# Snowdar/asv-subtools

Hardware: NVIDIA H100
Metric: frames/sec x-vector extraction (80-d fbank) (higher is better)
Workload: dtype f32 (bf16x3 split operands on wgmma, fp32 accumulate in registers)

## Files before the change

### asv_subtools_b200/csrc/ptx.cuh

```cuda
#pragma once
#include <cuda_runtime.h>
#include <cuda.h>
#include <stdint.h>

namespace xvb {

#ifndef XVB_WATCHDOG
#define XVB_WATCHDOG 1
#endif

__device__ __forceinline__ uint32_t smem_u32(const void* p) {
  return static_cast<uint32_t>(__cvta_generic_to_shared(p));
}

__device__ __forceinline__ uint32_t lane_id() {
  uint32_t l;
  asm volatile("mov.u32 %0, %%laneid;" : "=r"(l));
  return l;
}

__device__ __forceinline__ bool elect_one() {
  uint32_t pred = 0;
  asm volatile(
      "{\n\t"
// ... 48 lines not shown
      : "=r"(ok)
      : "r"(smem_u32(bar)), "r"(parity), "r"(1000000u)
      : "memory");
  return ok != 0;
}
__device__ __forceinline__ void mbar_wait(uint64_t* bar, uint32_t parity) {
#if XVB_WATCHDOG
  uint32_t spins = 0;
  while (!mbar_try_wait(bar, parity)) {
    if (++spins > 4000u) {
#if XVB_WATCHDOG >= 2
      printf("xvb: mbarrier watchdog: block %d thread %d bar@%u parity %u\n", (int)blockIdx.x, (int)threadIdx.x,
             smem_u32(bar), parity);
#endif
      __trap();
    }
  }
#else
  while (!mbar_try_wait(bar, parity)) {
  }
#endif
}

__device__ __forceinline__ void tma_prefetch_desc(const CUtensorMap* m) {
  asm volatile("prefetch.tensormap [%0];" ::"l"(reinterpret_cast<uint64_t>(m)) : "memory");
}
__device__ __forceinline__ void tma_load_2d(void* smem, const CUtensorMap* m, uint64_t* bar, int c0, int c1) {
  asm volatile(
      "cp.async.bulk.tensor.2d.shared::cluster.global.mbarrier::complete_tx::bytes [%0], [%1, {%3, %4}], [%2];" ::"r"(
          smem_u32(smem)),
      "l"(reinterpret_cast<uint64_t>(m)), "r"(smem_u32(bar)), "r"(c0), "r"(c1)
      : "memory");
}
__device__ __forceinline__ void tma_load_3d(void* smem, const CUtensorMap* m, uint64_t* bar, int c0, int c1, int c2) {
  asm volatile(
      "cp.async.bulk.tensor.3d.shared::cluster.global.mbarrier::complete_tx::bytes [%0], [%1, {%3, %4, %5}], [%2];" ::
          "r"(smem_u32(smem)),
      "l"(reinterpret_cast<uint64_t>(m)), "r"(smem_u32(bar)), "r"(c0), "r"(c1), "r"(c2)
      : "memory");
}
__device__ __forceinline__ void tma_load_4d(void* smem, const CUtensorMap* m, uint64_t* bar, int c0, int c1, int c2, int c3) {
  asm volatile(
      "cp.async.bulk.tensor.4d.shared::cluster.global.mbarrier::complete_tx::bytes [%0], [%1, {%3, %4, %5, %6}], [%2];" ::
          "r"(smem_u32(smem)),
      "l"(reinterpret_cast<uint64_t>(m)), "r"(smem_u32(bar)), "r"(c0), "r"(c1), "r"(c2), "r"(c3)
      : "memory");
}
__device__ __forceinline__ void tma_store_3d(const CUtensorMap* m, uint32_t smem_addr, int c0, int c1, int c2) {
  asm volatile("cp.async.bulk.tensor.3d.global.shared::cta.bulk_group [%0, {%2, %3, %4}], [%1];" ::"l"(
                   reinterpret_cast<uint64_t>(m)),
               "r"(smem_addr), "r"(c0), "r"(c1), "r"(c2)
               : "memory");
}
__device__ __forceinline__ void tma_store_commit() { asm volatile("cp.async.bulk.commit_group;" ::: "memory"); }
template <int kPending>
__device__ __forceinline__ void tma_store_wait_read() {
  asm volatile("cp.async.bulk.wait_group.read %0;" ::"n"(kPending) : "memory");
}
template <int kPending>
__device__ __forceinline__ void tma_store_wait_done() {
  asm volatile("cp.async.bulk.wait_group %0;" ::"n"(kPending) : "memory");
}
__device__ __forceinline__ void st_shared_u32(uint32_t addr, uint32_t v) {
  asm volatile("st.shared.b32 [%0], %1;" ::"r"(addr), "r"(v) : "memory");
}
__device__ __forceinline__ float2 ld_shared_f2(uint32_t addr) {
  float2 v;
  asm volatile("ld.shared.v2.f32 {%0, %1}, [%2];" : "=f"(v.x), "=f"(v.y) : "r"(addr));
  return v;
}
__device__ __forceinline__ void wgmma_fence() { asm volatile("wgmma.fence.sync.aligned;" ::: "memory"); }
__device__ __forceinline__ void wgmma_commit() { asm volatile("wgmma.commit_group.sync.aligned;" ::: "memory"); }
template <int kPending>
__device__ __forceinline__ void wgmma_wait() {
  asm volatile("wgmma.wait_group.sync.aligned %0;" ::"n"(kPending) : "memory");
}
template <uint32_t kRegs>
__device__ __forceinline__ void setmaxnreg_dec() { asm volatile("setmaxnreg.dec.sync.aligned.u32 %0;" ::"n"(kRegs)); }
template <uint32_t kRegs>
__device__ __forceinline__ void setmaxnreg_inc() { asm volatile("setmaxnreg.inc.sync.aligned.u32 %0;" ::"n"(kRegs)); }
template <int R>
__device__ __forceinline__ void wgmma_fence_operands(float (&d)[R]) {
#pragma unroll
  for (int i = 0; i < R; ++i) asm volatile("" : "+f"(d[i])::"memory");
}

template <int N>
__device__ __forceinline__ void wgmma_bf16(float (&d)[N / 2], uint64_t desc_a, uint64_t desc_b, uint32_t scale_d);
template <>
__device__ __forceinline__ void wgmma_bf16<32>(float (&d)[16], uint64_t desc_a, uint64_t desc_b, uint32_t scale_d) {
  asm volatile(
      "{\n\t.reg .pred p;\n\tsetp.ne.b32 p, %18, 0;\n\t"
      "wgmma.mma_async.sync.aligned.m64n32k16.f32.bf16.bf16 {%0, %1, %2, %3, %4, %5, %6, %7, %8, %9, %10, %11, %12, %13, %14, %15}, %16, %17, p, 1, 1, 0, 0;\n\t}\n"
      : "+f"(d[0]), "+f"(d[1]), "+f"(d[2]), "+f"(d[3]), "+f"(d[4]), "+f"(d[5]), "+f"(d[6]), "+f"(d[7]), "+f"(d[8]), "+f"(d[9]), "+f"(d[10]), "+f"(d[11]), "+f"(d[12]), "+f"(d[13]), "+f"(d[14]), "+f"(d[15])
      : "l"(desc_a), "l"(desc_b), "r"(scale_d));
}
template <>
__device__ __forceinline__ void wgmma_bf16<64>(float (&d)[32], uint64_t desc_a, uint64_t desc_b, uint32_t scale_d) {
  asm volatile(
      "{\n\t.reg .pred p;\n\tsetp.ne.b32 p, %34, 0;\n\t"
      "wgmma.mma_async.sync.aligned.m64n64k16.f32.bf16.bf16 {%0, %1, %2, %3, %4, %5, %6, %7, %8, %9, %10, %11, %12, %13, %14, %15, %16, %17, %18, %19, %20, %21, %22, %23, %24, %25, %26, %27, %28, %29, %30, %31}, %32, %33, p, 1, 1, 0, 0;\n\t}\n"
      : "+f"(d[0]), "+f"(d[1]), "+f"(d[2]), "+f"(d[3]), "+f"(d[4]), "+f"(d[5]), "+f"(d[6]), "+f"(d[7]), "+f"(d[8]), "+f"(d[9]), "+f"(d[10]), "+f"(d[11]), "+f"(d[12]), "+f"(d[13]), "+f"(d[14]), "+f"(d[15]), "+f"(d[16]), "+f"(d[17]), "+f"(d[18]), "+f"(d[19]), "+f"(d[20]), "+f"(d[21]), "+f"(d[22]), "+f"(d[23]), "+f"(d[24]), "+f"(d[25]), "+f"(d[26]), "+f"(d[27]), "+f"(d[28]), "+f"(d[29]), "+f"(d[30]), "+f"(d[31])
      : "l"(desc_a), "l"(desc_b), "r"(scale_d));
}
template <>
__device__ __forceinline__ void wgmma_bf16<128>(float (&d)[64], uint64_t desc_a, uint64_t desc_b, uint32_t scale_d) {
// ... 18 lines not shown
```

### asv_subtools_b200/csrc/tdnn_gemm.cu

```cuda
#include <cuda.h>
#include <cuda_bf16.h>
#include <cuda_runtime.h>

#include <stdlib.h>

#include <mutex>

#include "common.cuh"
#include "ptx.cuh"

namespace xvb {

constexpr int kBlockM = 128;
constexpr int kBlockK = 64;
constexpr int kABytes = kBlockM * kBlockK * 2;
constexpr int kNumConsumers = 256;
constexpr int kProducerWarp = kNumConsumers / 32;
constexpr int kSlabBytes = 16384;
constexpr int kStagePlaneBytes = 64 * kBlockK * 2;
constexpr int kStageOutBytes = 2 * kStagePlaneBytes;
constexpr int kCoefBytes = 3 * kBlockK * 4;
constexpr int kEpiBytes = 2 * (kStageOutBytes + kCoefBytes);
static_assert(kEpiBytes >= kSlabBytes, "the histogram slab lives in the epilogue region");

template <int BLOCK_N, bool kHist, bool kSwish>
__host__ __device__ constexpr bool ping_pong() { return BLOCK_N == 128 && !kHist && !kSwish; }
template <int BLOCK_N, bool kHist, bool kSwish>
__host__ __device__ constexpr int gemm_threads() { return kNumConsumers + (ping_pong<BLOCK_N, kHist, kSwish>() ? 128 : 32); }
constexpr uint32_t kProducerRegs = 40, kConsumerRegs = 232;

struct TdnnGemmParams {
  int B, T, Cin, Cout;
  int Tb, Bb, num_t_blk, num_b_blk, num_n_blk, num_tiles;
  int ntaps, cin_p16, num_cblk;
  int ctx[XVB_MAX_TAPS];
  int flags;
  const float* bias;
  const float* scale;
  const float* shift;
  const float* row_bias;
  const float* utt_bias;
  long long ld_utt;
  int log2_tb;
  float* pool_partial;
  int num_src;
  int unit_first, unit_stride;
  unsigned long long* hist;
  const int* row_label;
  const int* col_label;
  float hist_lo, hist_inv_w;
  int hist_bins;
  int hist_sym;
  int hist_group, num_units;
  int k_slices, kb_per_slice;
  int group_ng, group_kg;
  int out_T;
  const int* lengths;
  int tma_store;
#ifdef XVB_TILE_TIMELINE
  unsigned long long* timeline;
  int timeline_tiles;
  int timeline_general;
#endif
  __nv_bfloat16* y_hi;
  __nv_bfloat16* y_lo;
  long long ldy;
  float* y_f32;
  long long ldyf;
};

template <int BLOCK_N, bool kPool, bool kHist>
__host__ __device__ constexpr bool staged_epilogue() { return !kPool && !kHist && BLOCK_N % kBlockK == 0; }

template <int BLOCK_N, bool kStagedEpi>
struct GemmCfg {
  static constexpr int kTailBytes = kStagedEpi ? kEpiBytes : kSlabBytes;
  static constexpr int kBBytes = BLOCK_N * kBlockK * 2;
  static constexpr int kStageBytes = 2 * kABytes + 2 * kBBytes;
  static constexpr int kStages = (192 * 1024) / kStageBytes > 6 ? 6 : (192 * 1024) / kStageBytes;
  static constexpr int kAccRegs = BLOCK_N / 2;
  static constexpr int kSmemBytes = kStages * kStageBytes + kTailBytes + 1024  + 256 ;
  static_assert(kSmemBytes <= 232448, "exceeds the 227 KB shared memory of an sm_90 CTA");
  static_assert(kStages >= 2, "need at least a double-buffered operand pipeline");
};

template <bool kHist>
__device__ __forceinline__ bool decode_tile(const TdnnGemmParams& p, int tile, int& m_unit, int& n_blk, int& slice) {
  slice = 0;
  if constexpr (!kHist) {
    if (p.k_slices > 1) { slice = tile % p.k_slices; tile /= p.k_slices; }
    m_unit = p.unit_first + (tile / p.num_n_blk) * p.unit_stride;
    n_blk = tile % p.num_n_blk;
    return true;
  } else {
    const int per_band = p.num_n_blk * p.hist_group;
    const int band = tile / per_band, r = tile - band * per_band;
    n_blk = r / p.hist_group;
    const int mi = band * p.hist_group + (r - n_blk * p.hist_group);
    m_unit = 2 * (p.unit_first + (mi >> 1) * p.unit_stride) + (mi & 1);
    return mi < 2 * p.num_units && !(p.hist_sym && n_blk < m_unit);
  }
}

__device__ __forceinline__ void chan_merge(float& n, float& mean, float& m2, float nb, float meanb, float m2b) {
  const float tot = n + nb;
  if (tot > 0.f) {
    const float d = meanb - mean, wb = nb / tot;
    mean = fmaf(d, wb, mean);
    m2 += m2b + d * d * n * wb;
  }
  n = tot;
}

__device__ __noinline__ float epi_tanh(float v) { return tanhf(v); }
__device__ __noinline__ float epi_sigmoid(float v) { return 1.f / (1.f + expf(-v)); }

__device__ __noinline__ void epi_zero_row(const TdnnGemmParams& p, long long grow, long long frow, int c_begin, int c_end) {
  for (int c = c_begin; c < c_end; c += 8) {
    const bool has1 = c + 1 < p.Cout;
    if (p.y_hi) {
      if (has1) {
        *reinterpret_cast<uint32_t*>(p.y_hi + grow * p.ldy + c) = 0u;
        *reinterpret_cast<uint32_t*>(p.y_lo + grow * p.ldy + c) = 0u;
      } else {
        p.y_hi[grow * p.ldy + c] = __float2bfloat16(0.f);
        p.y_lo[grow * p.ldy + c] = __float2bfloat16(0.f);
      }
    }
    if (p.y_f32) {
      float* df = p.y_f32 + frow * p.ldyf + c;
      if (has1) *reinterpret_cast<float2*>(df) = make_float2(0.f, 0.f);
      else *df = 0.f;
    }
  }
}

#ifdef XVB_TILE_TIMELINE
#define XVB_TL(...) __VA_ARGS__
constexpr int kTimelineHead = 8, kTimelineRec = 8;
static unsigned long long* g_timeline = nullptr;
static int g_timeline_tiles = 0;
static bool g_timeline_direct = false;
__device__ __forceinline__ unsigned long long global_timer() {
  unsigned long long t;
  asm volatile("mov.u64 %0, %%globaltimer;" : "=l"(t));
  return t;
}
#else
#define XVB_TL(...)
#endif

template <int BLOCK_N, bool kPool, bool kHist, bool kSwish = false>
__global__ void __launch_bounds__(gemm_threads<BLOCK_N, kHist, kSwish>(), 1)
tdnn_gemm_bf16x3_kernel(const __grid_constant__ CUtensorMap map_a_hi, const __grid_constant__ CUtensorMap map_a_lo,
                        const __grid_constant__ CUtensorMap map_a2_hi, const __grid_constant__ CUtensorMap map_a2_lo,
                        const __grid_constant__ CUtensorMap map_w_hi, const __grid_constant__ CUtensorMap map_w_lo,
                        const __grid_constant__ CUtensorMap map_y_hi, const __grid_constant__ CUtensorMap map_y_lo,
                        const __grid_constant__ TdnnGemmParams p) {
  constexpr bool kStaged = staged_epilogue<BLOCK_N, kPool, kHist>();
  using Cfg = GemmCfg<BLOCK_N, kStaged>;
  constexpr int kStages = Cfg::kStages;
  constexpr int kBBytes = Cfg::kBBytes;
  constexpr int kStageBytes = Cfg::kStageBytes;
  static_assert(!kPool || BLOCK_N == kBlockM, "fused pooling: 128 channels x 128 frames per tile");
  constexpr bool kPingPong = ping_pong<BLOCK_N, kHist, kSwish>();
  constexpr int kHalves = kPingPong ? 2 : 1;
  constexpr int kReleaseWarps = kPingPong ? 4 : kNumConsumers / 32;

  extern __shared__ uint8_t smem_raw[];
  uint8_t* smem = reinterpret_cast<uint8_t*>((reinterpret_cast<uintptr_t>(smem_raw) + 1023) & ~uintptr_t(1023));
  uint8_t* slab_base = smem + kStages * kStageBytes;
  uint64_t* full_bar = reinterpret_cast<uint64_t*>(slab_base + Cfg::kTailBytes);
  uint64_t* empty_bar = full_bar + kStages;

  const int warp = threadIdx.x >> 5;
  const int lane = threadIdx.x & 31;

  if (warp == kProducerWarp && lane == 0) {
    tma_prefetch_desc(&map_a_hi);
    tma_prefetch_desc(&map_a_lo);
    tma_prefetch_desc(&map_w_hi);
    tma_prefetch_desc(&map_w_lo);
    if (kStaged && p.tma_store) {
      tma_prefetch_desc(&map_y_hi);
      tma_prefetch_desc(&map_y_lo);
    }
    for (int i = 0; i < kStages; ++i) {
      mbar_init(&full_bar[i], 1);
      mbar_init(&empty_bar[i], kReleaseWarps);
    }
    fence_barrier_init();
  }
  __syncthreads();
  asm volatile("griddepcontrol.wait;" ::: "memory");
  asm volatile("fence.proxy.async;" ::: "memory");

  const int num_kblk = p.num_src * p.ntaps * p.num_cblk;

  if (warp >= kProducerWarp) {
    if constexpr (kPingPong) setmaxnreg_dec<kProducerRegs>();
    if (warp == kProducerWarp && lane == 0) {
      int stage = 0;
      uint32_t phase = 0;
      for (int tile = blockIdx.x; tile < p.num_tiles; tile += gridDim.x) {
        int m_unit, n_blk, slice;
        if (!decode_tile<kHist>(p, tile, m_unit, n_blk, slice)) continue;
        const int cb_begin = slice * p.kb_per_slice;
        const int cb_end = p.k_slices > 1 ? min(p.num_cblk, cb_begin + p.kb_per_slice) : p.num_cblk;
        const int b0 = (m_unit / p.num_t_blk) * p.Bb, t0 = (m_unit % p.num_t_blk) * p.Tb;
        const int n0 = n_blk * BLOCK_N;
        const int a_c0 = p.group_ng ? (n0 / p.group_ng) * p.group_kg : 0;
        for (int src = 0; src < p.num_src; ++src) {
          const CUtensorMap* ma_hi = src == 0 ? &map_a_hi : &map_a2_hi;
          const CUtensorMap* ma_lo = src == 0 ? &map_a_lo : &map_a2_lo;
          for (int tap = 0; tap < p.ntaps; ++tap) {
            const int tt = t0 + p.ctx[tap];
            for (int cb = cb_begin; cb < cb_end; ++cb) {
              mbar_wait(&empty_bar[stage], phase ^ 1);
              uint8_t* s = smem + stage * kStageBytes;
              const int kw = tap * p.cin_p16 + cb * kBlockK;
              mbar_expect_tx(&full_bar[stage], kStageBytes);
              tma_load_3d(s, ma_hi, &full_bar[stage], a_c0 + cb * kBlockK, tt, b0);
              tma_load_3d(s + kABytes, ma_lo, &full_bar[stage], a_c0 + cb * kBlockK, tt, b0);
              tma_load_2d(s + 2 * kABytes, &map_w_hi, &full_bar[stage], kw, n0);
              tma_load_2d(s + 2 * kABytes + kBBytes, &map_w_lo, &full_bar[stage], kw, n0);
              if (++stage == kStages) { stage = 0; phase ^= 1; }
            }
          }
        }
      }
    }
    return;
  }

  if constexpr (kPingPong) setmaxnreg_inc<kConsumerRegs>();
  const int wg = warp >> 2;
  const int q4 = lane & 3;
  const int row_base = kPingPong ? 0 : 64 * wg;
  const int row0 = row_base + 16 * (warp & 3) + (lane >> 2);
  const int etid = threadIdx.x;
  const bool relu = (p.flags & XVB_RELU) != 0;
  const bool bn = (p.flags & XVB_BN) != 0;
  const bool act_sigmoid = (p.flags & XVB_SIGMOID) != 0;
  const bool act_tanh = (p.flags & XVB_TANH) != 0;
  const float relu_floor = relu ? 0.f : -INFINITY;
  float acc[kHalves][Cfg::kAccRegs];
#pragma unroll
  for (int hh = 0; hh < kHalves; ++hh)
#pragma unroll
    for (int i = 0; i < Cfg::kAccRegs; ++i) acc[hh][i] = 0.f;
  auto half_down = [&]() {
#pragma unroll
    for (int i = 0; i < Cfg::kAccRegs; ++i) acc[0][i] = acc[kHalves - 1][i];
  };
  int stage = 0;
  uint32_t phase = 0;
  uint32_t it = 0;

  uint32_t h_below[2] = {0u, 0u}, h_above[2] = {0u, 0u};
  const uint32_t hslab = smem_u32(slab_base);
  auto hist_flush = [&]() {
    asm volatile("bar.sync 1, 256;" ::: "memory");
#pragma unroll
    for (int c = 0; c < 2; ++c) {
      if (h_below[c]) asm volatile("red.shared.add.u32 [%0], %1;" ::"r"(hslab + (c * p.hist_bins) * 4), "r"(h_below[c]) : "memory");
      if (h_above[c]) asm volatile("red.shared.add.u32 [%0], %1;" ::"r"(hslab + (c * p.hist_bins + p.hist_bins - 1) * 4), "r"(h_above[c]) : "memory");
      h_below[c] = 0u; h_above[c] = 0u;
    }
    asm volatile("bar.sync 1, 256;" ::: "memory");
    for (int e = etid; e < 2 * p.hist_bins; e += kNumConsumers) {
      uint32_t c;
      asm volatile("ld.shared.u32 %0, [%1];" : "=r"(c) : "r"(hslab + e * 4) : "memory");
      if (c) {
        atomicAdd(p.hist + e, (unsigned long long)c);
        asm volatile("st.shared.u32 [%0], %1;" ::"r"(hslab + e * 4), "r"(0u) : "memory");
      }
    }
    asm volatile("bar.sync 1, 256;" ::: "memory");
  };
  if constexpr (kHist) {
    for (int e = etid; e < 2 * p.hist_bins; e += kNumConsumers)
      asm volatile("st.shared.u32 [%0], %1;" ::"r"(hslab + e * 4), "r"(0u) : "memory");
    asm volatile("bar.sync 1, 256;" ::: "memory");
  }

  XVB_TL(
    long long tl_start = 0, tl_first = 0, tl_issued = 0, tl_retired = 0, tl_wait = 0;
    unsigned long long* tl_cta = p.timeline ? p.timeline + (size_t)blockIdx.x * (kTimelineHead + (size_t)kTimelineRec * p.timeline_tiles) : nullptr;
    if (tl_cta && threadIdx.x == 0) { tl_cta[0] = global_timer(); tl_cta[1] = (unsigned long long)clock64(); }
  )
  int tj = 0;
  XVB_TL(auto tl_flush = [&]() {
    if (tl_cta && (threadIdx.x & 127) == 0 && tj < p.timeline_tiles) {
      unsigned long long* r = tl_cta + kTimelineHead + (size_t)kTimelineRec * tj;
      r[0] = (unsigned long long)tl_start; r[1] = (unsigned long long)tl_first; r[2] = (unsigned long long)tl_issued;
      r[3] = (unsigned long long)tl_retired; r[4] = (unsigned long long)clock64(); r[5] = (unsigned long long)tl_wait;
      r[6] = (unsigned long long)wg; r[7] = 1ull;
    }
  };)
  for (int tile = blockIdx.x; tile < p.num_tiles; tile += gridDim.x, ++tj) {
    int m_unit, n_blk, slice;
    if (!decode_tile<kHist>(p, tile, m_unit, n_blk, slice)) continue;
    int kb_begin = 0, kb_end = num_kblk;
    if (p.k_slices > 1) {
      kb_begin = slice * p.kb_per_slice;
      kb_end = min(num_kblk, kb_begin + p.kb_per_slice);
    }
    if constexpr (kPingPong) {
      if ((tj & 1) != wg) {
        stage += kb_end - kb_begin;
        phase ^= (uint32_t)(stage / kStages) & 1u;
        stage %= kStages;
        continue;
      }
      if (tj > 0) asm volatile("bar.sync %0, 256;" ::"r"(2 + wg) : "memory");
    }
    ++it;
    XVB_TL(tl_start = clock64(); tl_wait = 0;)
    auto stage_before = [&]() { return stage == 0 ? kStages - 1 : stage - 1; };
    for (int kb = kb_begin; kb < kb_end; ++kb) {
      XVB_TL(const long long tl_w0 = clock64();)
      mbar_wait(&full_bar[stage], phase);
      XVB_TL(const long long tl_w1 = clock64(); tl_wait += tl_w1 - tl_w0; tl_first = kb == kb_begin ? tl_w1 : tl_first;)
      const uint32_t sa = smem_u32(smem + stage * kStageBytes);
      const uint64_t dx_hi = make_sw128_desc(sa), dx_lo = make_sw128_desc(sa + kABytes);
      const uint64_t dw_hi = make_sw128_desc(sa + 2 * kABytes), dw_lo = make_sw128_desc(sa + 2 * kABytes + kBBytes);
      const uint64_t da_hi = kPool ? dw_hi : dx_hi, da_lo = kPool ? dw_lo : dx_lo;
      const uint64_t db_hi = kPool ? dx_hi : dw_hi, db_lo = kPool ? dx_lo : dw_lo;
      wgmma_fence();
#pragma unroll
      for (int s = 0; s < kBlockK / 16; ++s) {
        const uint64_t koff = (uint64_t)(s * 32 >> 4);
#pragma unroll
        for (int hh = 0; hh < kHalves; ++hh) {
          const uint64_t m_off = (uint64_t)((row_base + 64 * hh) * 128 >> 4);
          wgmma_bf16<BLOCK_N>(acc[hh], da_lo + m_off + koff, db_hi + koff, s == 0 ? (uint32_t)(kb != kb_begin) : 1u);
          wgmma_bf16<BLOCK_N>(acc[hh], da_hi + m_off + koff, db_lo + koff, 1);
          wgmma_bf16<BLOCK_N>(acc[hh], da_hi + m_off + koff, db_hi + koff, 1);
        }
      }
      wgmma_commit();
      wgmma_wait<1>();
      if (kb != kb_begin && lane == 0) mbar_arrive(&empty_bar[stage_before()]);
      if (++stage == kStages) { stage = 0; phase ^= 1; }
    }
    if (kPingPong && tile + gridDim.x < p.num_tiles) asm volatile("bar.arrive %0, 256;" ::"r"(3 - wg) : "memory");
    XVB_TL(tl_issued = clock64();)
    wgmma_wait<0>();
    XVB_TL(tl_retired = clock64();)
#pragma unroll
    for (int hh = 0; hh < kHalves; ++hh) wgmma_fence_operands(acc[hh]);
    if (kb_end > kb_begin && lane == 0) mbar_arrive(&empty_bar[stage_before()]);

    const int b0 = (m_unit / p.num_t_blk) * p.Bb, t0 = (m_unit % p.num_t_blk) * p.Tb;
    const int n0 = n_blk * BLOCK_N;

    if constexpr (kPool) {
      int nv = p.T - t0;
      nv = nv < 0 ? 0 : (nv > p.Tb ? p.Tb : nv);
      const int tblk = m_unit % p.num_t_blk;
      const int gl = p.Tb < 8 ? p.Tb : 8;
#pragma unroll 1
      for (int hh = 0; hh < kHalves; ++hh) {
      if (hh > 0) half_down();
      int b0h = b0, nvh = nv;
      asm volatile("" : "+r"(b0h), "+r"(nvh));
      if (p.Tb == 8 && nvh == 8 XVB_TL(&& !p.timeline_general)) {
#pragma unroll
        for (int h = 0; h < 2; ++h) {
          const int cch = n0 + row0 + 64 * hh + 8 * h;
          const bool cvalid = cch < p.Cout;
          const float bias_c = (cvalid && p.bias) ? __ldg(p.bias + cch) : 0.f;
          const float scale_c = (cvalid && bn) ? __ldg(p.scale + cch) : 1.f;
          const float shift_c = (cvalid && bn) ? __ldg(p.shift + cch) : 0.f;
          float* dst0 = p.pool_partial + ((long long)tblk * p.B + b0h) * (2LL * p.Cout) + cch;
          const bool writer = cvalid && q4 == 0;
#pragma unroll
          for (int i = 0; i < BLOCK_N / 8; ++i) {
            const float x0 = fmaf(fmaxf(acc[0][4 * i + 2 * h] + bias_c, relu_floor), scale_c, shift_c);
            const float x1 = fmaf(fmaxf(acc[0][4 * i + 2 * h + 1] + bias_c, relu_floor), scale_c, shift_c);
            float mean = 0.5f * (x0 + x1) + 0.f;
            float m2 = 0.5f * (x0 - x1) * (x0 - x1);
            float d = __shfl_xor_sync(0xffffffffu, mean, 1) - mean;
            float m2b = __shfl_xor_sync(0xffffffffu, m2, 1);
            mean = fmaf(d, 0.5f, mean);
            m2 += m2b + d * d * 2.f * 0.5f;
            d = __shfl_xor_sync(0xffffffffu, mean, 2) - mean;
            m2b = __shfl_xor_sync(0xffffffffu, m2, 2);
            mean = fmaf(d, 0.5f, mean);
            m2 += m2b + d * d * 4.f * 0.5f;
            if (writer && b0h + i < p.B) {
              float* dst = dst0 + (long long)i * (2LL * p.Cout);
              dst[0] = mean;
              dst[p.Cout] = m2;
            }
          }
        }
        continue;
      }
#pragma unroll
      for (int h = 0; h < 2; ++h) {
        const int cch = n0 + row0 + 64 * hh + 8 * h;
        const bool cvalid = cch < p.Cout;
        const float bias_c = (cvalid && p.bias) ? __ldg(p.bias + cch) : 0.f;
        const float scale_c = (cvalid && bn) ? __ldg(p.scale + cch) : 1.f;
        const float shift_c = (cvalid && bn) ? __ldg(p.shift + cch) : 0.f;
        auto emit = [&](int col, float mean, float m2) {
          const int bb = b0h + (col >> p.log2_tb);
          if (cvalid && bb < p.B) {
            float* dst = p.pool_partial + ((long long)tblk * p.B + bb) * (2LL * p.Cout) + cch;
            dst[0] = mean;
            dst[p.Cout] = m2;
          }
        };
        float rn = 0.f, rmean = 0.f, rm2 = 0.f;
#pragma unroll
        for (int i = 0; i < BLOCK_N / 8; ++i) {
          const int col = 8 * i + 2 * q4;
          const float x0 = fmaf(fmaxf(acc[0][4 * i + 2 * h] + bias_c, relu_floor), scale_c, shift_c);
          const float x1 = fmaf(fmaxf(acc[0][4 * i + 2 * h + 1] + bias_c, relu_floor), scale_c, shift_c);
          if (p.Tb == 1) {
            if (nvh > 0) { emit(col, x0, 0.f); emit(col + 1, x1, 0.f); }
            continue;
          }
          const int j = col & (p.Tb - 1);
          const bool v0 = j < nvh, v1 = j + 1 < nvh;
          const float pn = (float)v0 + (float)v1;
          const float pm = v1 ? 0.5f * (x0 + x1) : (v0 ? x0 : 0.f);
          const float pm2 = v1 ? 0.5f * (x0 - x1) * (x0 - x1) : 0.f;
          chan_merge(rn, rmean, rm2, pn, pm, pm2);
          if (((col - 2 * q4 + 8) & (p.Tb - 1)) == 0) {
            if (gl >= 4) chan_merge(rn, rmean, rm2, __shfl_xor_sync(0xffffffffu, rn, 1),
                                    __shfl_xor_sync(0xffffffffu, rmean, 1), __shfl_xor_sync(0xffffffffu, rm2, 1));
            if (gl >= 8) chan_merge(rn, rmean, rm2, __shfl_xor_sync(0xffffffffu, rn, 2),
                                    __shfl_xor_sync(0xffffffffu, rmean, 2), __shfl_xor_sync(0xffffffffu, rm2, 2));
            if (((2 * q4) & (gl - 1)) == 0 && rn > 0.f) emit(col & ~(p.Tb - 1), rmean, rm2);
            rn = 0.f; rmean = 0.f; rm2 = 0.f;
          }
        }
      }
      }
      XVB_TL(tl_flush();)
      continue;
    }

    if constexpr (kHist) {
      const float top = (float)(p.hist_bins - 2);
#pragma unroll
      for (int h = 0; h < 2; ++h) {
        const int row = row0 + 8 * h;
        const int b = b0 + (row >> p.log2_tb), t = t0 + (row & (p.Tb - 1));
        const bool valid = (b < p.B) && (t < p.T);
        const float rbias = (p.row_bias && valid) ? __ldg(p.row_bias + (long long)b * p.T + t) : 0.f;
        const int lab_r = valid ? __ldg(p.row_label + b) : -1;
#pragma unroll
        for (int i = 0; i < BLOCK_N / 8; ++i) {
#pragma unroll
          for (int e = 0; e < 2; ++e) {
            const int c = n0 + 8 * i + 2 * q4 + e;
            const bool in = c < p.Cout;
            const uint32_t ok = (valid && in && (!p.hist_sym || c > b)) ? 1u : 0u;
            const float sc = acc[0][4 * i + 2 * h + e] + ((in && p.bias) ? __ldg(p.bias + c) : 0.f) + rbias;
            const float x = (sc - p.hist_lo) * p.hist_inv_w;
            const uint32_t cls = (in && __ldg(p.col_label + c) == lab_r) ? 1u : 0u;
            const uint32_t bl = x < 0.f ? ok : 0u;
            const uint32_t ab = !(x < top) ? ok : 0u;
            h_below[0] += bl & (cls ^ 1u); h_below[1] += bl & cls;
            h_above[0] += ab & (cls ^ 1u); h_above[1] += ab & cls;
            if (ok & ~(bl | ab))
              asm volatile("red.shared.add.u32 [%0], %1;" ::"r"(hslab + ((int)cls * p.hist_bins + 1 + (int)x) * 4), "r"(1u) : "memory");
          }
        }
      }
      if ((it & 0x3fffu) == 0) hist_flush();
      continue;
    }

    if constexpr (kStaged) {
      if (p.tma_store) {
        int tid = threadIdx.x;
        asm volatile("" : "+r"(tid));
        const int wgo = tid >> 7, wtid = tid & 127, q4o = tid & 3;
        const int prow = 16 * ((tid >> 5) & 3) + ((tid & 31) >> 2);
        const uint32_t stg = smem_u32(slab_base) + wgo * kStageOutBytes;
        const uint32_t coefs = smem_u32(slab_base) + 2 * kStageOutBytes + wgo * kCoefBytes;
        const int ebar = 4 + wgo;
        const uint32_t coef = coefs + 8 * q4o;
        const uint32_t my = stg + (uint32_t)prow * 128u + ((uint32_t)(prow & 7) << 4) + 4u * q4o;
#pragma unroll 1
        for (int hh = 0; hh < kHalves; ++hh) {
          if (hh > 0) half_down();
          const int hrow = (kPingPong ? 0 : 64 * wgo) + 64 * hh;
          uint32_t keep[2];
#pragma unroll
          for (int r = 0; r < 2; ++r) {
            const int row = hrow + prow + 8 * r;
            const int b = b0 + (row >> p.log2_tb), t = t0 + (row & (p.Tb - 1));
            keep[r] = (p.lengths && b < p.B && t >= __ldg(p.lengths + b)) ? 0u : 0xffffffffu;
          }
#pragma unroll
          for (int cr = 0; cr < BLOCK_N / kBlockK; ++cr) {
            const int c0 = n0 + kBlockK * cr;
            if (c0 >= p.Cout) break;
            if (wtid == 0) tma_store_wait_read<0>();
            if (wtid < kBlockK) {
              const int c = c0 + wtid;
              const bool in = c < p.Cout;
              st_shared_f32(coefs + 4 * wtid, (in && p.bias) ? __ldg(p.bias + c) : 0.f);
              st_shared_f32(coefs + 4 * (kBlockK + wtid), (in && bn) ? __ldg(p.scale + c) : 1.f);
              st_shared_f32(coefs + 4 * (2 * kBlockK + wtid), (in && bn) ? __ldg(p.shift + c) : 0.f);
            }
            asm volatile("bar.sync %0, 128;" ::"r"(ebar) : "memory");
#pragma unroll
            for (int i = 0; i < kBlockK / 8; ++i) {
              const float2 bias_c = ld_shared_f2(coef + 32 * i), scale_c = ld_shared_f2(coef + 32 * i + 4 * kBlockK),
                           shift_c = ld_shared_f2(coef + 32 * i + 8 * kBlockK);
              const float bias_e[2] = {bias_c.x, bias_c.y}, scale_e[2] = {scale_c.x, scale_c.y},
                          shift_e[2] = {shift_c.x, shift_c.y};
#pragma unroll
              for (int r = 0; r < 2; ++r) {
                float x[2] = {acc[0][4 * (8 * cr + i) + 2 * r], acc[0][4 * (8 * cr + i) + 2 * r + 1]};
#pragma unroll
                for (int e = 0; e < 2; ++e) {
                  float v = x[e] + bias_e[e] + 0.f;
                  v = fmaxf(v, relu_floor);
                  if constexpr (kSwish) v = v / (1.f + expf(-v));
                  if (bn) v = fmaf(v, scale_e[e], shift_e[e]);
                  if (act_tanh) v = epi_tanh(v);
                  if (act_sigmoid) v = epi_sigmoid(v);
                  x[e] = v;
                }
                __nv_bfloat16 h0, l0, h1, l1;
                split_bf16(x[0], h0, l0);
                split_bf16(x[1], h1, l1);
                const uint32_t at = (my ^ ((uint32_t)i << 4)) + 1024u * r;
                st_shared_u32(at, pack_bf16x2(h0, h1) & keep[r]);
                st_shared_u32(at + kStagePlaneBytes, pack_bf16x2(l0, l1) & keep[r]);
              }
            }
            fence_proxy_async();
            asm volatile("bar.sync %0, 128;" ::"r"(ebar) : "memory");
            if (wtid == 0) {
              const int hb = b0 + (hrow >> p.log2_tb), ht = t0 + (hrow & (p.Tb - 1));
              tma_store_3d(&map_y_hi, stg, c0, ht, hb);
              tma_store_3d(&map_y_lo, stg + kStagePlaneBytes, c0, ht, hb);
              tma_store_commit();
            }
          }
        }
        XVB_TL(tl_flush();)
        continue;
      }
    }
    if constexpr (!kPool && !kHist) {
#pragma unroll 1
      for (int hh = 0; hh < kHalves; ++hh) {
      if (hh > 0) half_down();
      constexpr int kRows = 2;
      bool live[kRows];
      float rbias[kRows];
      const float* ub[kRows];
      long long grow[kRows], frow[kRows];
#pragma unroll
      for (int r = 0; r < kRows; ++r) {
        const int row = row0 + 64 * hh + 8 * r;
        const int b = b0 + (row >> p.log2_tb), t = t0 + (row & (p.Tb - 1));
        live[r] = b < p.B && t < p.T;
        grow[r] = (long long)b * p.T + t;
        frow[r] = (long long)b * p.out_T + t + slice;
        if (live[r] && p.lengths && t >= __ldg(p.lengths + b)) {
          epi_zero_row(p, grow[r], frow[r], n0 + 2 * q4, min(n0 + BLOCK_N, p.Cout));
          live[r] = false;
        }
        rbias[r] = (live[r] && p.row_bias) ? __ldg(p.row_bias + grow[r]) : 0.f;
        ub[r] = (live[r] && p.utt_bias) ? p.utt_bias + (long long)b * p.ld_utt : nullptr;
      }
#pragma unroll
      for (int i = 0; i < BLOCK_N / 8; ++i) {
        const int c = n0 + 8 * i + 2 * q4;
        if (c >= p.Cout) break;
        const bool has1 = c + 1 < p.Cout;
        float bias_c[2], scale_c[2], shift_c[2];
#pragma unroll
        for (int e = 0; e < 2; ++e) {
          const bool in = e == 0 || has1;
          bias_c[e] = (in && p.bias) ? __ldg(p.bias + c + e) : 0.f;
          scale_c[e] = (in && bn) ? __ldg(p.scale + c + e) : 1.f;
          shift_c[e] = (in && bn) ? __ldg(p.shift + c + e) : 0.f;
        }
#pragma unroll
        for (int r = 0; r < kRows; ++r) {
          if (!live[r]) continue;
          float x[2] = {acc[0][4 * i + 2 * r], acc[0][4 * i + 2 * r + 1]};
#pragma unroll
          for (int e = 0; e < 2; ++e) {
            if (e == 1 && !has1) break;
            float v = x[e] + bias_c[e] + rbias[r];
            if (ub[r]) v += __ldg(ub[r] + c + e);
            v = fmaxf(v, relu_floor);
            if constexpr (kSwish) v = v / (1.f + expf(-v));
            if (bn) v = fmaf(v, scale_c[e], shift_c[e]);
            if (act_tanh) v = epi_tanh(v);
            if (act_sigmoid) v = epi_sigmoid(v);
            x[e] = v;
          }
          if (p.y_hi) {
            __nv_bfloat16 h0, l0, h1, l1;
            split_bf16(x[0], h0, l0);
            split_bf16(x[1], h1, l1);
            __nv_bfloat16* dh = p.y_hi + grow[r] * p.ldy + c;
            __nv_bfloat16* dl = p.y_lo + grow[r] * p.ldy + c;
            if (has1) {
              *reinterpret_cast<uint32_t*>(dh) = pack_bf16x2(h0, h1);
              *reinterpret_cast<uint32_t*>(dl) = pack_bf16x2(l0, l1);
            } else {
              *dh = h0;
              *dl = l0;
            }
          }
          if (p.y_f32) {
            float* df = p.y_f32 + frow[r] * p.ldyf + c;
            if (has1) *reinterpret_cast<float2*>(df) = make_float2(x[0], x[1]);
            else *df = x[0];
          }
        }
      }
      }
      XVB_TL(tl_flush();)
    }
  }
  if constexpr (kHist) hist_flush();
  if constexpr (kStaged) {
    if (p.tma_store && (threadIdx.x & 127) == 0) tma_store_wait_done<0>();
  }
  XVB_TL(if (tl_cta && (threadIdx.x & 127) == 0) { tl_cta[2 + 2 * wg] = global_timer(); tl_cta[3 + 2 * wg] = (unsigned long long)clock64(); })
}

__global__ void segment_reduce_kernel(const float* __restrict__ part, int S, int B, int Cout, const float* __restrict__ bias,
                                      const float* __restrict__ scale, const float* __restrict__ shift, int flags,
                                      float* __restrict__ y_f32, long long ldyf, __nv_bfloat16* __restrict__ y_hi,
                                      __nv_bfloat16* __restrict__ y_lo, long long ldy) {
  asm volatile("griddepcontrol.wait;" ::: "memory");
  const long long idx = blockIdx.x * (long long)blockDim.x + threadIdx.x;
  if (idx >= (long long)B * Cout) return;
  const int b = (int)(idx / Cout), c = (int)(idx - (long long)b * Cout);
  const float* src = part + (long long)b * S * Cout + c;
  float x = src[0];
  for (int s = 1; s < S; ++s) x += src[(long long)s * Cout];
  x += bias ? bias[c] : 0.f;
  if (flags & XVB_RELU) x = fmaxf(x, 0.f);
  if (flags & XVB_BN) x = fmaf(x, scale[c], shift[c]);
  if (flags & XVB_TANH) x = tanhf(x);
  if (flags & XVB_SIGMOID) x = 1.f / (1.f + expf(-x));
  if (y_f32) y_f32[(long long)b * ldyf + c] = x;
  if (y_hi) {
    __nv_bfloat16 h, l;
    split_bf16(x, h, l);
    y_hi[(long long)b * ldy + c] = h;
    y_lo[(long long)b * ldy + c] = l;
  }
}

typedef CUresult (*PFN_encodeTiled)(CUtensorMap*, CUtensorMapDataType, cuuint32_t, void*, const cuuint64_t*,
                                    const cuuint64_t*, const cuuint32_t*, const cuuint32_t*, CUtensorMapInterleave,
                                    CUtensorMapSwizzle, CUtensorMapL2promotion, CUtensorMapFloatOOBfill);

static PFN_encodeTiled get_encode() {
  static PFN_encodeTiled fn = nullptr;
  static std::once_flag once;
  std::call_once(once, [] {
    void* p = nullptr;
    cudaDriverEntryPointQueryResult q;
    if (cudaGetDriverEntryPoint("cuTensorMapEncodeTiled", &p, cudaEnableDefault, &q) == cudaSuccess &&
        q == cudaDriverEntryPointSuccess)
      fn = reinterpret_cast<PFN_encodeTiled>(p);
  });
  return fn;
}

int make_tensor_map(CUtensorMap* m, const void* base, int esize, int rank, const unsigned long long* dims,
                    const unsigned long long* strides_bytes, const unsigned* box, int swizzle_bytes) {
  PFN_encodeTiled enc = get_encode();
  if (!enc) { set_error("cuTensorMapEncodeTiled entry point not available"); return XVB_ECUDA; }
  cuuint64_t d[5], st[4];
  cuuint32_t bx[5], es[5];
  for (int i = 0; i < rank; ++i) { d[i] = dims[i]; bx[i] = box[i]; es[i] = 1; }
  for (int i = 0; i + 1 < rank; ++i) st[i] = strides_bytes[i];
  const CUtensorMapSwizzle sw = swizzle_bytes == 128 ? CU_TENSOR_MAP_SWIZZLE_128B
                               : swizzle_bytes == 64 ? CU_TENSOR_MAP_SWIZZLE_64B : CU_TENSOR_MAP_SWIZZLE_NONE;
  CUresult r = enc(m, esize == 2 ? CU_TENSOR_MAP_DATA_TYPE_BFLOAT16 : CU_TENSOR_MAP_DATA_TYPE_FLOAT32, rank,
                   const_cast<void*>(base), d, st, bx, es, CU_TENSOR_MAP_INTERLEAVE_NONE, sw,
                   CU_TENSOR_MAP_L2_PROMOTION_L2_256B, CU_TENSOR_MAP_FLOAT_OOB_FILL_NONE);
  if (r != CUDA_SUCCESS) { set_error("cuTensorMapEncodeTiled(rank %d) failed: %d", rank, (int)r); return XVB_ECUDA; }
  return XVB_OK;
}

static int make_frame_map(CUtensorMap* m, const void* base, int C, int T, int B, long long ld, int Tb, int Bb,
                          long long batch_stride = 0) {
  PFN_encodeTiled enc = get_encode();
  if (!enc) { set_error("cuTensorMapEncodeTiled entry point not available"); return XVB_ECUDA; }
  cuuint64_t dims[3] = {(cuuint64_t)C, (cuuint64_t)T, (cuuint64_t)B};
  cuuint64_t strides[2] = {(cuuint64_t)ld * 2, batch_stride ? (cuuint64_t)batch_stride * 2 : (cuuint64_t)ld * 2 * (cuuint64_t)T};
  cuuint32_t box[3] = {(cuuint32_t)kBlockK, (cuuint32_t)Tb, (cuuint32_t)Bb};
  cuuint32_t estr[3] = {1, 1, 1};
  CUresult r = enc(m, CU_TENSOR_MAP_DATA_TYPE_BFLOAT16, 3, const_cast<void*>(base), dims, strides, box, estr,
                   CU_TENSOR_MAP_INTERLEAVE_NONE, CU_TENSOR_MAP_SWIZZLE_128B, CU_TENSOR_MAP_L2_PROMOTION_L2_256B,
                   CU_TENSOR_MAP_FLOAT_OOB_FILL_NONE);
  if (r != CUDA_SUCCESS) { set_error("cuTensorMapEncodeTiled(frame map C=%d T=%d B=%d ld=%lld) failed: %d", C, T, B, ld, (int)r); return XVB_ECUDA; }
  return XVB_OK;
}

static int make_store_map(CUtensorMap* m, const void* base, int Cout, int T, int B, long long ld, int Tb) {
  const int box_t = Tb < 64 ? Tb : 64;
  const unsigned long long dims[3] = {(unsigned long long)Cout, (unsigned long long)T, (unsigned long long)B};
  const unsigned long long strides[2] = {(unsigned long long)ld * 2, (unsigned long long)ld * 2 * (unsigned long long)T};
  const unsigned box[3] = {(unsigned)kBlockK, (unsigned)box_t, (unsigned)(64 / box_t)};
  return make_tensor_map(m, base, 2, 3, dims, strides, box, 128);
}

static int make_weight_map(CUtensorMap* m, const void* base, long long K, int Cout, int block_n) {
  PFN_encodeTiled enc = get_encode();
  if (!enc) { set_error("cuTensorMapEncodeTiled entry point not available"); return XVB_ECUDA; }
  cuuint64_t dims[2] = {(cuuint64_t)K, (cuuint64_t)Cout};
  cuuint64_t strides[1] = {(cuuint64_t)K * 2};
  cuuint32_t box[2] = {(cuuint32_t)kBlockK, (cuuint32_t)block_n};
  cuuint32_t estr[2] = {1, 1};
  CUresult r = enc(m, CU_TENSOR_MAP_DATA_TYPE_BFLOAT16, 2, const_cast<void*>(base), dims, strides, box, estr,
                   CU_TENSOR_MAP_INTERLEAVE_NONE, CU_TENSOR_MAP_SWIZZLE_128B, CU_TENSOR_MAP_L2_PROMOTION_L2_256B,
                   CU_TENSOR_MAP_FLOAT_OOB_FILL_NONE);
  if (r != CUDA_SUCCESS) { set_error("cuTensorMapEncodeTiled(weight map K=%lld Cout=%d) failed: %d", K, Cout, (int)r); return XVB_ECUDA; }
  return XVB_OK;
}

static void choose_m_tile(int B, int T, int* Tb_out, int* Bb_out, int max_tb = 128) {
  if (T == 1) {
    *Tb_out = 1;
    *Bb_out = 128;
    return;
  }
  long long best = -1;
  int bt = max_tb;
  for (int Tb = max_tb; Tb >= 1; Tb >>= 1) {
    const int Bb = 128 / Tb;
    const long long rows = (long long)((T + Tb - 1) / Tb) * Tb * ((B + Bb - 1) / Bb) * Bb;
    if (best < 0 || rows < best) { best = rows; bt = Tb; }
  }
  *Tb_out = bt;
  *Bb_out = 128 / bt;
}

struct GemmPlan {
  CUtensorMap ma_hi, ma_lo, ma2_hi, ma2_lo, mw_hi, mw_lo, my_hi, my_lo;
  TdnnGemmParams p;
  int (*launch)(const GemmPlan&, const TdnnGemmParams&, cudaStream_t) = nullptr;
  int grid = 0;
  int pdl = 1;
  bool reduce = false;
  const float* r_bias = nullptr; const float* r_scale = nullptr; const float* r_shift = nullptr;
  int r_flags = 0;
  float* r_y_f32 = nullptr; long long r_ldyf = 0;
  __nv_bfloat16* r_y_hi = nullptr; __nv_bfloat16* r_y_lo = nullptr; long long r_ldy = 0;
};

template <int BLOCK_N, bool kPool, bool kHist, bool kSwish>
static int launch_inst(const GemmPlan& pl, const TdnnGemmParams& p, cudaStream_t stream) {
  using Cfg = GemmCfg<BLOCK_N, staged_epilogue<BLOCK_N, kPool, kHist>()>;
  XVB_ENSURE_DYN_SMEM((tdnn_gemm_bf16x3_kernel<BLOCK_N, kPool, kHist, kSwish>), Cfg::kSmemBytes);
  cudaLaunchConfig_t cfg{};
  cfg.gridDim = dim3(pl.grid);
  cfg.blockDim = dim3(gemm_threads<BLOCK_N, kHist, kSwish>());
  cfg.dynamicSmemBytes = Cfg::kSmemBytes;
  cfg.stream = stream;
  cudaLaunchAttribute attr[1];
  attr[0].id = cudaLaunchAttributeProgrammaticStreamSerialization;
  attr[0].val.programmaticStreamSerializationAllowed = 1;
  cfg.attrs = attr;
  cfg.numAttrs = pl.pdl ? 1 : 0;
  XVB_CUDA(cudaLaunchKernelEx(&cfg, tdnn_gemm_bf16x3_kernel<BLOCK_N, kPool, kHist, kSwish>, pl.ma_hi, pl.ma_lo, pl.ma2_hi,
                              pl.ma2_lo, pl.mw_hi, pl.mw_lo, pl.my_hi, pl.my_lo, p));
  XVB_LAUNCH_CHECK();
  return XVB_OK;
}

template <int BLOCK_N, bool kPool = false, bool kHist = false, bool kSwish = false>
static int prepare_gemm(GemmPlan& pl, const void* w_hi, const void* w_lo) {
  TdnnGemmParams& p = pl.p;
  const long long K = (long long)p.ntaps * p.cin_p16;
  int rc = make_weight_map(&pl.mw_hi, w_hi, K, p.Cout, BLOCK_N);
  if (rc) return rc;
  rc = make_weight_map(&pl.mw_lo, w_lo, K, p.Cout, BLOCK_N);
  if (rc) return rc;
  p.num_n_blk = (p.Cout + BLOCK_N - 1) / BLOCK_N;
  p.tma_store = staged_epilogue<BLOCK_N, kPool, kHist>() && p.y_hi && !p.y_f32 && p.k_slices == 1 && !p.row_bias && !p.utt_bias &&
                p.Cout % 8 == 0;
  XVB_TL(if (g_timeline_direct) p.tma_store = 0;)
  if (p.tma_store) {
    if ((rc = make_store_map(&pl.my_hi, p.y_hi, p.Cout, p.T, p.B, p.ldy, p.Tb))) return rc;
    if ((rc = make_store_map(&pl.my_lo, p.y_lo, p.Cout, p.T, p.B, p.ldy, p.Tb))) return rc;
  } else {
    pl.my_hi = pl.mw_hi; pl.my_lo = pl.mw_lo;
  }
  const int all_m_units = kHist ? (p.num_t_blk * p.num_b_blk + 1) / 2 : p.num_t_blk * p.num_b_blk;
  if (p.unit_first >= all_m_units) { pl.launch = nullptr; return XVB_OK; }
  const int num_m_units = (all_m_units - p.unit_first + p.unit_stride - 1) / p.unit_stride;
  p.num_units = num_m_units;
  p.hist_group = 8;
  const long long tiles = kHist ? (long long)((2 * num_m_units + p.hist_group - 1) / p.hist_group) * p.hist_group * p.num_n_blk
                                : (long long)num_m_units * p.num_n_blk * (p.k_slices > 1 ? p.k_slices : 1);
  XVB_CHECK_ARG(tiles < (1ll << 31), "xvb_tdnn_affine: %d x %d tiles exceed one launch", num_m_units, p.num_n_blk);
  p.num_tiles = (int)tiles;
  p.out_T = p.k_slices > 1 ? p.k_slices : p.T;
  const int sms = sm_count();
  pl.grid = p.num_tiles < sms ? p.num_tiles : sms;
  static const int pdl = getenv("XVB_PDL") ? atoi(getenv("XVB_PDL")) : 1;
  pl.pdl = pdl;
  pl.launch = &launch_inst<BLOCK_N, kPool, kHist, kSwish>;
  return XVB_OK;
}

static int splitk_slices(const xvb_tdnn_args_t& a, bool has_hist, int* kb_per_slice) {
  const int num_cblk = (a.Cin + kBlockK - 1) / kBlockK;
  *kb_per_slice = num_cblk;
  const int splitk = getenv("XVB_SPLITK") ? atoi(getenv("XVB_SPLITK")) : 1;
  if (!(splitk && a.T == 1 && a.ntaps == 1 && !a.x2_hi && !a.pool_partial && !has_hist && !a.row_bias && !a.utt_bias &&
        !(a.flags & XVB_SWISH) && a.groups <= 1 &&
        a.B <= 1024 && num_cblk >= 24 && a.Cout % 4 == 0))
    return 1;
  int S = num_cblk / 6;
  S = S > 8 ? 8 : S;
  *kb_per_slice = (num_cblk + S - 1) / S;
  return (num_cblk + *kb_per_slice - 1) / *kb_per_slice;
}

}

using namespace xvb;

size_t xvb::gemm_plan_scratch_bytes(const xvb_tdnn_args_t& a, const TrialHist* th) {
  int kb;
  const int S = splitk_slices(a, th != nullptr, &kb);
  return S > 1 ? (size_t)a.B * S * a.Cout * sizeof(float) : 0;
}

int xvb::gemm_plan_build(GemmPlan** out, const xvb_tdnn_args_t& a, const TrialHist* th, void* scratch) {
  int rc = require_sm90();
  if (rc) return rc;
  *out = nullptr;
  const int B = a.B, T = a.T, Cin = a.Cin, Cout = a.Cout, ntaps = a.ntaps;
  XVB_CHECK_ARG(a.x_hi && a.x_lo && a.w_hi && a.w_lo, "xvb_tdnn_affine: null operand pointer");
// ... 204 lines not shown
```

Baseline: 34.48 million.

## Stage pooling partial statistics in shared memory and write them with TMA stores

The pooling epilogue (Tb==8) now writes per-tile mean/M2 partials into the shared-memory epilogue slab instead of scattering them to global memory from individual threads. One thread per warpgroup then issues a 4D bulk tensor store through a new tensor map over the pool_partial buffer. This replaces many strided scalar global stores with one async bulk copy per tile, at the cost of extra shared memory for the pooling variant and extra barrier and store-wait synchronisation. Timeline instrumentation records epilogue phase times when the timeline build flag is on.

```diff
diff --git a/asv_subtools_b200/csrc/ptx.cuh b/asv_subtools_b200/csrc/ptx.cuh
--- a/asv_subtools_b200/csrc/ptx.cuh
+++ b/asv_subtools_b200/csrc/ptx.cuh
@@ -124,6 +124,12 @@
                "r"(smem_addr), "r"(c0), "r"(c1), "r"(c2)
                : "memory");
 }
+__device__ __forceinline__ void tma_store_4d(const CUtensorMap* m, uint32_t smem_addr, int c0, int c1, int c2, int c3) {
+  asm volatile("cp.async.bulk.tensor.4d.global.shared::cta.bulk_group [%0, {%2, %3, %4, %5}], [%1];" ::"l"(
+                   reinterpret_cast<uint64_t>(m)),
+               "r"(smem_addr), "r"(c0), "r"(c1), "r"(c2), "r"(c3)
+               : "memory");
+}
 __device__ __forceinline__ void tma_store_commit() { asm volatile("cp.async.bulk.commit_group;" ::: "memory"); }
 template <int kPending>
 __device__ __forceinline__ void tma_store_wait_read() {
diff --git a/asv_subtools_b200/csrc/tdnn_gemm.cu b/asv_subtools_b200/csrc/tdnn_gemm.cu
--- a/asv_subtools_b200/csrc/tdnn_gemm.cu
+++ b/asv_subtools_b200/csrc/tdnn_gemm.cu
@@ -72,9 +72,9 @@
 template <int BLOCK_N, bool kPool, bool kHist>
 __host__ __device__ constexpr bool staged_epilogue() { return !kPool && !kHist && BLOCK_N % kBlockK == 0; }
 
-template <int BLOCK_N, bool kStagedEpi>
+template <int BLOCK_N, bool kPool, bool kHist>
 struct GemmCfg {
-  static constexpr int kTailBytes = kStagedEpi ? kEpiBytes : kSlabBytes;
+  static constexpr int kTailBytes = (staged_epilogue<BLOCK_N, kPool, kHist>() || kPool) ? kEpiBytes : kSlabBytes;
   static constexpr int kBBytes = BLOCK_N * kBlockK * 2;
   static constexpr int kStageBytes = 2 * kABytes + 2 * kBBytes;
   static constexpr int kStages = (192 * 1024) / kStageBytes > 6 ? 6 : (192 * 1024) / kStageBytes;
@@ -137,7 +137,7 @@
 
 #ifdef XVB_TILE_TIMELINE
 #define XVB_TL(...) __VA_ARGS__
-constexpr int kTimelineHead = 8, kTimelineRec = 8;
+constexpr int kTimelineHead = 8, kTimelineRec = 12;
 static unsigned long long* g_timeline = nullptr;
 static int g_timeline_tiles = 0;
 static bool g_timeline_direct = false;
@@ -158,7 +158,7 @@
                         const __grid_constant__ CUtensorMap map_y_hi, const __grid_constant__ CUtensorMap map_y_lo,
                         const __grid_constant__ TdnnGemmParams p) {
   constexpr bool kStaged = staged_epilogue<BLOCK_N, kPool, kHist>();
-  using Cfg = GemmCfg<BLOCK_N, kStaged>;
+  using Cfg = GemmCfg<BLOCK_N, kPool, kHist>;
   constexpr int kStages = Cfg::kStages;
   constexpr int kBBytes = Cfg::kBBytes;
   constexpr int kStageBytes = Cfg::kStageBytes;
@@ -181,7 +181,7 @@
     tma_prefetch_desc(&map_a_lo);
     tma_prefetch_desc(&map_w_hi);
     tma_prefetch_desc(&map_w_lo);
-    if (kStaged && p.tma_store) {
+    if ((kStaged || kPool) && p.tma_store) {
       tma_prefetch_desc(&map_y_hi);
       tma_prefetch_desc(&map_y_lo);
     }
@@ -286,6 +286,9 @@
 
   XVB_TL(
     long long tl_start = 0, tl_first = 0, tl_issued = 0, tl_retired = 0, tl_wait = 0;
+    long long tl_ep[4] = {0, 0, 0, 0};
+    long long tl_t = 0;
+    auto tl_mark = [&](int ph) { const long long t = clock64(); tl_ep[ph] += t - tl_t; tl_t = t; };
     unsigned long long* tl_cta = p.timeline ? p.timeline + (size_t)blockIdx.x * (kTimelineHead + (size_t)kTimelineRec * p.timeline_tiles) : nullptr;
     if (tl_cta && threadIdx.x == 0) { tl_cta[0] = global_timer(); tl_cta[1] = (unsigned long long)clock64(); }
   )
@@ -296,6 +299,7 @@
       r[0] = (unsigned long long)tl_start; r[1] = (unsigned long long)tl_first; r[2] = (unsigned long long)tl_issued;
       r[3] = (unsigned long long)tl_retired; r[4] = (unsigned long long)clock64(); r[5] = (unsigned long long)tl_wait;
       r[6] = (unsigned long long)wg; r[7] = 1ull;
+      for (int ph = 0; ph < 4; ++ph) r[8 + ph] = (unsigned long long)tl_ep[ph];
     }
   };)
   for (int tile = blockIdx.x; tile < p.num_tiles; tile += gridDim.x, ++tj) {
@@ -313,10 +317,13 @@
         stage %= kStages;
         continue;
       }
-      if (tj > 0) asm volatile("bar.sync %0, 256;" ::"r"(2 + wg) : "memory");
+      if (tj > 0) {
+        if (kPool && (threadIdx.x & 127) == 0) tma_store_wait_read<0>();
+        asm volatile("bar.sync %0, 256;" ::"r"(2 + wg) : "memory");
+      }
     }
     ++it;
-    XVB_TL(tl_start = clock64(); tl_wait = 0;)
+    XVB_TL(tl_start = clock64(); tl_wait = 0; tl_ep[0] = tl_ep[1] = tl_ep[2] = tl_ep[3] = 0;)
     auto stage_before = [&]() { return stage == 0 ? kStages - 1 : stage - 1; };
     for (int kb = kb_begin; kb < kb_end; ++kb) {
       XVB_TL(const long long tl_w0 = clock64();)
@@ -347,7 +354,7 @@
     if (kPingPong && tile + gridDim.x < p.num_tiles) asm volatile("bar.arrive %0, 256;" ::"r"(3 - wg) : "memory");
     XVB_TL(tl_issued = clock64();)
     wgmma_wait<0>();
-    XVB_TL(tl_retired = clock64();)
+    XVB_TL(tl_retired = clock64(); tl_t = tl_retired;)
 #pragma unroll
     for (int hh = 0; hh < kHalves; ++hh) wgmma_fence_operands(acc[hh]);
     if (kb_end > kb_begin && lane == 0) mbar_arrive(&empty_bar[stage_before()]);
@@ -365,7 +372,7 @@
       if (hh > 0) half_down();
       int b0h = b0, nvh = nv;
       asm volatile("" : "+r"(b0h), "+r"(nvh));
-      if (p.Tb == 8 && nvh == 8 XVB_TL(&& !p.timeline_general)) {
+      if (p.tma_store && p.Tb == 8 && nvh == 8 XVB_TL(&& !p.timeline_general)) {
 #pragma unroll
         for (int h = 0; h < 2; ++h) {
           const int cch = n0 + row0 + 64 * hh + 8 * h;
@@ -373,8 +380,10 @@
           const float bias_c = (cvalid && p.bias) ? __ldg(p.bias + cch) : 0.f;
           const float scale_c = (cvalid && bn) ? __ldg(p.scale + cch) : 1.f;
           const float shift_c = (cvalid && bn) ? __ldg(p.shift + cch) : 0.f;
-          float* dst0 = p.pool_partial + ((long long)tblk * p.B + b0h) * (2LL * p.Cout) + cch;
-          const bool writer = cvalid && q4 == 0;
+          int tid = threadIdx.x;
+          asm volatile("" : "+r"(tid));
+          const uint32_t dst0 = smem_u32(slab_base) + (tid >> 7) * kStageOutBytes +
+                                4 * (16 * ((tid >> 5) & 3) + ((tid & 31) >> 2) + 64 * hh + 8 * h);
 #pragma unroll
           for (int i = 0; i < BLOCK_N / 8; ++i) {
             const float x0 = fmaf(fmaxf(acc[0][4 * i + 2 * h] + bias_c, relu_floor), scale_c, shift_c);
@@ -389,13 +398,13 @@
             m2b = __shfl_xor_sync(0xffffffffu, m2, 2);
             mean = fmaf(d, 0.5f, mean);
             m2 += m2b + d * d * 4.f * 0.5f;
-            if (writer && b0h + i < p.B) {
-              float* dst = dst0 + (long long)i * (2LL * p.Cout);
-              dst[0] = mean;
-              dst[p.Cout] = m2;
+            if (q4 == 0) {
+              st_shared_f32(dst0 + 2 * 4 * BLOCK_N * i, mean);
+              st_shared_f32(dst0 + 2 * 4 * BLOCK_N * i + 4 * BLOCK_N, m2);
             }
           }
         }
+        XVB_TL(tl_mark(2);)
         continue;
       }
 #pragma unroll
@@ -440,6 +449,17 @@
         }
       }
       }
+      XVB_TL(tl_mark(2);)
+      if (p.tma_store && p.Tb == 8 && nv == 8 XVB_TL(&& !p.timeline_general)) {
+        fence_proxy_async();
+        asm volatile("bar.sync %0, 128;" ::"r"(4 + wg) : "memory");
+        XVB_TL(tl_mark(1);)
+        if ((threadIdx.x & 127) == 0) {
+          tma_store_4d(&map_y_hi, smem_u32(slab_base) + wg * kStageOutBytes, n0, 0, b0, tblk);
+          tma_store_commit();
+        }
+        XVB_TL(tl_mark(3);)
+      }
       XVB_TL(tl_flush();)
       continue;
     }
@@ -503,6 +523,7 @@
             const int c0 = n0 + kBlockK * cr;
             if (c0 >= p.Cout) break;
             if (wtid == 0) tma_store_wait_read<0>();
+            XVB_TL(tl_mark(0);)
             if (wtid < kBlockK) {
               const int c = c0 + wtid;
               const bool in = c < p.Cout;
@@ -511,6 +532,7 @@
               st_shared_f32(coefs + 4 * (2 * kBlockK + wtid), (in && bn) ? __ldg(p.shift + c) : 0.f);
             }
             asm volatile("bar.sync %0, 128;" ::"r"(ebar) : "memory");
+            XVB_TL(tl_mark(1);)
 #pragma unroll
             for (int i = 0; i < kBlockK / 8; ++i) {
               const float2 bias_c = ld_shared_f2(coef + 32 * i), scale_c = ld_shared_f2(coef + 32 * i + 4 * kBlockK),
@@ -538,6 +560,7 @@
                 st_shared_u32(at + kStagePlaneBytes, pack_bf16x2(l0, l1) & keep[r]);
               }
             }
+            XVB_TL(tl_mark(2);)
             fence_proxy_async();
             asm volatile("bar.sync %0, 128;" ::"r"(ebar) : "memory");
             if (wtid == 0) {
@@ -546,6 +569,7 @@
               tma_store_3d(&map_y_lo, stg + kStagePlaneBytes, c0, ht, hb);
               tma_store_commit();
             }
+            XVB_TL(tl_mark(3);)
           }
         }
         XVB_TL(tl_flush();)
@@ -630,7 +654,7 @@
     }
   }
   if constexpr (kHist) hist_flush();
-  if constexpr (kStaged) {
+  if constexpr (kStaged || kPool) {
     if (p.tma_store && (threadIdx.x & 127) == 0) tma_store_wait_done<0>();
   }
   XVB_TL(if (tl_cta && (threadIdx.x & 127) == 0) { tl_cta[2 + 2 * wg] = global_timer(); tl_cta[3 + 2 * wg] = (unsigned long long)clock64(); })
@@ -718,6 +742,13 @@
   return make_tensor_map(m, base, 2, 3, dims, strides, box, 128);
 }
 
+static int make_partial_map(CUtensorMap* m, const float* base, int Cout, int B, int nblk) {
+  const unsigned long long dims[4] = {(unsigned long long)Cout, 2ull, (unsigned long long)B, (unsigned long long)nblk};
+  const unsigned long long strides[3] = {4ull * Cout, 8ull * Cout, 8ull * Cout * (unsigned long long)B};
+  const unsigned box[4] = {(unsigned)kBlockM, 2u, 16u, 1u};
+  return make_tensor_map(m, base, 4, 4, dims, strides, box, 0);
+}
+
 static int make_weight_map(CUtensorMap* m, const void* base, long long K, int Cout, int block_n) {
   PFN_encodeTiled enc = get_encode();
   if (!enc) { set_error("cuTensorMapEncodeTiled entry point not available"); return XVB_ECUDA; }
@@ -764,7 +795,7 @@
 
 template <int BLOCK_N, bool kPool, bool kHist, bool kSwish>
 static int launch_inst(const GemmPlan& pl, const TdnnGemmParams& p, cudaStream_t stream) {
-  using Cfg = GemmCfg<BLOCK_N, staged_epilogue<BLOCK_N, kPool, kHist>()>;
+  using Cfg = GemmCfg<BLOCK_N, kPool, kHist>;
   XVB_ENSURE_DYN_SMEM((tdnn_gemm_bf16x3_kernel<BLOCK_N, kPool, kHist, kSwish>), Cfg::kSmemBytes);
   cudaLaunchConfig_t cfg{};
   cfg.gridDim = dim3(pl.grid);
@@ -793,8 +824,12 @@
   p.num_n_blk = (p.Cout + BLOCK_N - 1) / BLOCK_N;
   p.tma_store = staged_epilogue<BLOCK_N, kPool, kHist>() && p.y_hi && !p.y_f32 && p.k_slices == 1 && !p.row_bias && !p.utt_bias &&
                 p.Cout % 8 == 0;
+  if (kPool) p.tma_store = p.Tb == 8;
   XVB_TL(if (g_timeline_direct) p.tma_store = 0;)
-  if (p.tma_store) {
+  if (kPool && p.tma_store) {
+    if ((rc = make_partial_map(&pl.my_hi, p.pool_partial, p.Cout, p.B, p.num_t_blk))) return rc;
+    pl.my_lo = pl.mw_lo;
+  } else if (p.tma_store) {
     if ((rc = make_store_map(&pl.my_hi, p.y_hi, p.Cout, p.T, p.B, p.ldy, p.Tb))) return rc;
     if ((rc = make_store_map(&pl.my_lo, p.y_lo, p.Cout, p.T, p.B, p.ldy, p.Tb))) return rc;
   } else {
```

Result: faster. 35.69 million (median of 6 runs) (+3.5%).
